# jacobstern/volume-viz

Hardware: AMD Instinct MI355X
Metric: Msamples/s (rays x steps), 1024^3 f32 volume @1080p (higher is better)
Workload: dtype f32

## Files before the change

### volume-viz_amd/csrc/vv_api.cpp

```cpp
#include "../../include/volviz.h"
#include "vv_kernels.h"

#include <hip/hip_runtime.h>
#include <climits>
#include <cmath>
#include <cstdio>
#include <cstdlib>
#include <cstring>
#include <string>
#include <algorithm>
#include <vector>

using namespace vv;

struct vv_knobs {
    int tile_log2w = -1, xcd_band = -1, unroll = -1, lds_reserve = -1, lds_reserve_phong = -1;
    int bricked = -1, zpair = -1, zfast = -1, force_big = 0;
    int block_w = -1, tail = -1, rect = -1, lpt = -1, lpt_run = -1, phong_bricks = -1;
    static int geti(const char *name, int dflt) { const char *e = getenv(name); return e ? atoi(e) : dflt; }
    void read()
    {
        tile_log2w = geti("VV_TILE_LOG2W", -1); xcd_band = geti("VV_XCD_BAND", -1); unroll = geti("VV_UNROLL", -1);
        lds_reserve = geti("VV_LDS_RESERVE", -1); lds_reserve_phong = geti("VV_LDS_RESERVE_PHONG", -1);
        bricked = geti("VV_BRICKED", -1); zpair = geti("VV_ZPAIR", -1);
        block_w = geti("VV_BLOCK_W", -1); tail = geti("VV_TAIL", -1);
        zfast = geti("VV_ZFAST", -1); force_big = getenv("VV_FORCE_BIG") != nullptr;
        rect = geti("VV_RECT", -1); lpt = geti("VV_LPT", -1); lpt_run = geti("VV_LPT_RUN", -1); phong_bricks = geti("VV_PHONG_BRICKS", -1);
    }
};

struct vv_context {
    int device = 0;
    vv_knobs knobs;
    hipStream_t stream = nullptr;
    hipEvent_t ev0 = nullptr, ev1 = nullptr;
    bool timed = false, time_frames = true;
    void *d_vol = nullptr; size_t vol_bytes = 0; int vtype = VV_VOXEL_U8; int nx = 0, ny = 0, nz = 0;
    size_t row_pitch = 0, slice_pitch = 0, alloc_bytes = 0;
    void *d_bricks = nullptr; bool bricks_valid = false, bricks_failed = false; uint32_t b_sy = 0, b_sz64 = 0; size_t bricks_bytes = 0;
    void *d_zpair = nullptr; bool zpair_valid = false; uint32_t zp_row = 0, zp_slab = 0; size_t zpair_bytes = 0;
    void *d_zfast = nullptr; bool zfast_valid = false, zfast_failed = false; uint32_t zf_row = 0; uint64_t zf_slice = 0; size_t zfast_bytes = 0;
    void *d_xpair = nullptr; bool xpair_valid = false, xpair_failed = false; uint32_t xp_row = 0, xp_slab = 0; size_t xpair_bytes = 0;
    size_t layout_budget_bytes = 0; bool build_in_render = true;
    unsigned long long frame_no = 0, last_used[4] = {0, 0, 0, 0};
    unsigned long long builds_in_render = 0;
    float last_density = 1e9f;
    float4 *d_tf = nullptr; bool tf_gray = false; bool have_tf = false;
    bool tf_alpha_unit = false;
    float *d_rad = nullptr; size_t rad_cap = 0;
// ... 594 lines not shown
    }
    launch_build_xpair(c->vtype, c->d_zfast, c->zf_row, c->zf_slice, c->d_xpair, c->nx, c->ny, c->nz, st);
    if (hipGetLastError() != hipSuccess ||
        hipMemsetAsync((char *)c->d_xpair + xb, 0, 32, st) != hipSuccess || hipStreamSynchronize(st) != hipSuccess) {
        (void)hipGetLastError(); (void)hipFree(c->d_xpair); c->d_xpair = nullptr; c->xpair_failed = true;
        return false;
    }
    c->xp_row = rb; c->xp_slab = sb; c->xpair_bytes = xb; c->xpair_valid = true;
    return true;
}

static VolumeView view_of(const vv_context *c)
{
    VolumeView V;
    const uint32_t vsz = c->vtype == VV_VOXEL_F32 ? 4 : 1;
    V.data = c->d_vol; V.nx = c->nx; V.ny = c->ny; V.nz = c->nz;
    (void)vsz;
    V.row_bytes = (uint32_t)c->row_pitch;
    V.slice_bytes = (uint32_t)c->slice_pitch;
    V.big = c->slice_pitch * (size_t)c->nz > (1ull << 32) || V.slice_bytes >= (1u << 24) || c->knobs.force_big;
    V.bricks = nullptr; V.b_sy = 0; V.b_sz64 = 0;
    V.zpair = nullptr; V.zp_row_bytes = 0; V.zp_slab_bytes = 0;
    V.zfast = nullptr; V.zf_row_bytes = 0; V.zf_slice_bytes = 0;
    return V;
}

static inline float vlen_h(float x, float y, float z) { return sqrtf(x * x + y * y + z * z); }

static int camera_basis(vv_context *c, FrameParams &P, const camera_params *cam, const vv_ray_source *rays, int W, int H)
{
    float lx = rays->look[0], ly = rays->look[1], lz = rays->look[2];
    float ll = vlen_h(lx, ly, lz);
    if (!(ll > 0.f)) return fail(c, VV_ERR_INVALID, "vv_render: look vector is zero");
    lx /= ll; ly /= ll; lz /= ll;
    float ux = rays->up[0], uy = rays->up[1], uz = rays->up[2];
    float sx = ly * uz - lz * uy, sy = lz * ux - lx * uz, sz = lx * uy - ly * ux;
    float sl = vlen_h(sx, sy, sz);
    if (!(sl > 0.f)) return fail(c, VV_ERR_INVALID, "vv_render: up vector is parallel to look");
    sx /= sl; sy /= sl; sz /= sl;
    float vx = sy * lz - sz * ly, vy = sz * lx - sx * lz, vz = sx * ly - sy * lx;
    float vl = vlen_h(vx, vy, vz);
    vx /= vl; vy /= vl; vz /= vl;
    P.look[0] = lx; P.look[1] = ly; P.look[2] = lz;
    P.side[0] = sx; P.side[1] = sy; P.side[2] = sz;
    P.up[0] = vx; P.up[1] = vy; P.up[2] = vz;
    float aspect = rays->aspect > 0.f ? rays->aspect : (float)W / (float)H;
// ... 73 lines not shown
    if (use_bricks) use_bricks = c->build_in_render ? ensure_bricks(c, st) : c->bricks_valid;
    if (use_bricks) {
        c->last_used[CP_BRICKS] = c->frame_no;
        A.V.bricks = c->d_bricks; A.V.b_sy = c->b_sy; A.V.b_sz64 = c->b_sz64;
        if (!k_unroll) A.unroll = 2;
        if (!k_reserve) A.lds_reserve = beyond_caches ? big_reserve : 36000;
    }
    bool use_zpair = !use_bricks && A.strips.tile_log2w == 5 && !shading->phongShading &&
                     (c->vtype == VV_VOXEL_U8 || c->vol_bytes <= (512ull << 20));
    if (K.zpair >= 0) use_zpair = K.zpair != 0 && !use_bricks;
    if (use_zfast) use_zpair = false;
    if (use_zpair) use_zpair = c->build_in_render ? ensure_zpair(c, st) : c->zpair_valid;
    if (use_zpair) { c->last_used[CP_ZPAIR] = c->frame_no; A.V.zpair = c->d_zpair; A.V.zp_row_bytes = c->zp_row; A.V.zp_slab_bytes = c->zp_slab; }
    A.xpair = false;
    if (use_zfast && !shading->phongShading && K.zpair != 0 && (c->vtype == VV_VOXEL_U8 || c->vol_bytes <= (512ull << 20)) &&
        (c->build_in_render ? ensure_xpair(c, st) : c->xpair_valid)) {
        A.xpair = true; c->last_used[CP_XPAIR] = c->frame_no;
        A.V.zpair = c->d_xpair; A.V.zp_row_bytes = c->xp_row; A.V.zp_slab_bytes = c->xp_slab;
    }
    c->builds_in_render += ((unsigned long long)c->bricks_valid + c->zpair_valid + c->zfast_valid + c->xpair_valid > builds_before)
                           ? ((unsigned long long)c->bricks_valid + c->zpair_valid + c->zfast_valid + c->xpair_valid - builds_before) : 0;
    A.lds_reserve_phong = c->vol_bytes > (8ull << 30) ? 40000 : ((beyond_caches && density > 3.5f && !use_bricks) ? 30000 : 13000);
    if (K.lds_reserve_phong >= 0 && K.lds_reserve_phong <= 146 * 1024) A.lds_reserve_phong = K.lds_reserve_phong;
    c->last_density = density;
    return beyond_caches;
}

static bool screen_rect(const MarchArgs &A, int W, int H, double *xmin, double *xmax, double *ymin, double *ymax)
{
    const FrameParams &P = A.P;
    double lo[2] = {INFINITY, INFINITY}, hi[2] = {-INFINITY, -INFINITY}, dmin = INFINITY, ext = 0.0;
    for (int a = 0; a < 3; ++a) ext = std::max(ext, (double)fabsf(P.cam_pos[a]) + (double)P.scale[a]);
    for (int k = 0; k < 8; ++k) {
        const double v[3] = {((k & 1) ? P.scale[0] : -P.scale[0]) - (double)P.cam_pos[0], ((k & 2) ? P.scale[1] : -P.scale[1]) - (double)P.cam_pos[1],
                             ((k & 4) ? P.scale[2] : -P.scale[2]) - (double)P.cam_pos[2]};
        const double depth = v[0] * P.look[0] + v[1] * P.look[1] + v[2] * P.look[2];
        if (!(depth > 1e-3 * ext)) return false;
        dmin = std::min(dmin, depth);
        const double sx = (v[0] * P.side[0] + v[1] * P.side[1] + v[2] * P.side[2]) / depth, sy = (v[0] * P.up[0] + v[1] * P.up[1] + v[2] * P.up[2]) / depth;
        const double px = (sx / P.tan_half_x + 1.0) * 0.5 * W - 0.5, py = (sy / P.tan_half_y + 1.0) * 0.5 * H - 0.5;
        lo[0] = std::min(lo[0], px); hi[0] = std::max(hi[0], px); lo[1] = std::min(lo[1], py); hi[1] = std::max(hi[1], py);
    }
    const double ang = 1e-4 * ext / dmin;
    const double mx = 1.0 + ang / (2.0 * P.tan_half_x / W), my = 1.0 + ang / (2.0 * P.tan_half_y / H);
    if (!std::isfinite(lo[0] + hi[0] + lo[1] + hi[1] + mx + my) || mx > W || my > H) return false;
    *xmin = lo[0] - mx; *xmax = hi[0] + mx; *ymin = lo[1] - my; *ymax = hi[1] + my;
// ... 213 lines not shown
        if (!whole) HIPCHK(c, hipMemcpyAsync(d_out, rgba_out, fb, hipMemcpyHostToDevice, st));
    }
    A.pixels = (uint32_t *)d_out;
    if (((uintptr_t)d_out & 3) != 0) return fail(c, VV_ERR_INVALID, "vv_render: output buffer must be 4-byte aligned");

    if (A.instr) HIPCHK(c, hipMemsetAsync(c->d_counter, 0, 16 * sizeof(unsigned long long), st));
#ifdef VV_TIMELINE
    { const char *e = getenv("VV_TIMELINE_PTR"); A.I.timeline = e ? (unsigned long long *)strtoull(e, nullptr, 0) : nullptr; }
#endif
    c->counter_valid = A.instr;
    {
        const int layout = A.xpair ? 5 : A.V.zfast ? 4 : (A.V.bricks ? 2 : (A.V.zpair ? 3 : ((A.V.big || (A.phong && beyond_caches)) ? 1 : 0)));
        const int v[8] = {A.strips.tile_log2w, A.strips.blk_log2w, A.unroll, A.phong ? A.lds_reserve_phong : A.lds_reserve, layout, have_basis ? 1 : 0,
                          (int)fminf(density * 1000.f, 2e9f), A.phong ? 1 : 0};
        memcpy(c->last_launch, v, sizeof v);
    }
    if (c->time_frames) HIPCHK(c, hipEventRecord(c->ev0, st));
    if (A.phong) {
        if (A.fill_outside) { A.rad_out = nullptr; launch_rad(A, st); }
        if (A.xpair) launch_raymarch_xpair(A, st); else if (A.V.zfast) launch_raymarch_zfast(A, st); else if (A.V.bricks) { if (beyond_caches) launch_raymarch_bricked(A, st); else launch_raymarch_bricked_cached(A, st); } else if (A.V.zpair) launch_raymarch_zpair(A, st); else if (A.V.big || beyond_caches) launch_raymarch_big(A, st); else launch_raymarch(A, st);
    } else if (A.strips.n_strips > 0) {
        if (W >= 2 && H >= 2) launch_rad(A, st);
        if (A.xpair) launch_raymarch_xpair(A, st);
        else if (A.V.zfast) launch_raymarch_zfast(A, st);
        else if (A.V.bricks) { if (beyond_caches) launch_raymarch_bricked(A, st); else launch_raymarch_bricked_cached(A, st); }
        else if (A.V.zpair) launch_raymarch_zpair(A, st);
        else if (A.V.big) launch_raymarch_big(A, st);
        else launch_raymarch(A, st);
    }
    if (c->time_frames) HIPCHK(c, hipEventRecord(c->ev1, st));
    HIPCHK(c, hipGetLastError());
    c->timed = c->time_frames;
    if (!out_on_device) {
        if (whole) HIPCHK(c, hipMemcpy2DAsync(rgba_out, (size_t)W * 4, d_out, (size_t)W * 4, (size_t)(W - 1) * 4, (size_t)(H - 1), hipMemcpyDeviceToHost, st));
        else HIPCHK(c, hipMemcpyAsync(rgba_out, d_out, fb, hipMemcpyDeviceToHost, st));
        HIPCHK(c, hipStreamSynchronize(st));
    } else if (!stream) {
        HIPCHK(c, hipStreamSynchronize(st));
    }
    return VV_OK;
}

int vv_first_pass(vv_context *c, int W, int H, const camera_params *cam, const vv_ray_source *rays,
                  uint8_t *front, uint8_t *back, int out_on_device, void *stream)
{
    if (!c) return fail(nullptr, VV_ERR_INVALID, "vv_first_pass: NULL context");
    if (!cam || !rays || !front || !back || W < 1 || H < 1) return fail(c, VV_ERR_INVALID, "vv_first_pass: bad argument");
    if (rays->mode != VV_RAYS_ANALYTIC) return fail(c, VV_ERR_INVALID, "vv_first_pass: needs an analytic ray source");
    for (int a = 0; a < 3; ++a)
// ... 211 lines not shown
```

### volume-viz_amd/csrc/vv_device.h

```cpp
#pragma once
#include <hip/hip_runtime.h>
#include <stdint.h>
#include "../../include/volviz.h"

namespace vv {

constexpr int   kCacheDepth = 32;
constexpr float kChunkSteps = 30.f;
constexpr int   kSlab = 14;
constexpr int   kBlock = 16;
constexpr float kSqrt3 = 1.73205081f;
constexpr float kEps = 1e-6f;

struct f3 { float x, y, z; };
__device__ __forceinline__ f3 mk3(float x, float y, float z) { return f3{x, y, z}; }

struct VolumeView {
    const void *data;
    int nx, ny, nz;
    uint32_t row_bytes;
    uint32_t slice_bytes;
    int big;
    const void *bricks;
    uint32_t b_sy;
    uint32_t b_sz64;
    const void *zpair;
    uint32_t zp_row_bytes;
    uint32_t zp_slab_bytes;
    const void *zfast;
    uint32_t zf_row_bytes;
    uint64_t zf_slice_bytes;
};
template <int VOXEL> struct BrickGeom;
#ifndef VV_BRICK_XLOG2
#define VV_BRICK_XLOG2 2
#endif
#ifndef VV_BRICK_HALO
#define VV_BRICK_HALO 1
#endif
#ifndef VV_BRICK_ZLOG2
#define VV_BRICK_ZLOG2 2
#endif
#ifndef VV_BRICK_X7
#define VV_BRICK_X7 0
#endif
#ifndef VV_BRICK_EXTRA
#define VV_BRICK_EXTRA 0
#endif
#if VV_BRICK_X7
template <> struct BrickGeom<VV_VOXEL_F32> { static constexpr uint32_t xlog2 = 0, bx = 7, halo = 1, row = 32,
                                             zlog2 = VV_BRICK_ZLOG2, bz = 1u << zlog2, rows = 4 * bz, brick = rows * row + VV_BRICK_EXTRA; };
#else
template <> struct BrickGeom<VV_VOXEL_F32> { static constexpr uint32_t xlog2 = VV_BRICK_XLOG2, bx = 1u << xlog2, halo = VV_BRICK_HALO, row = (bx + halo) * 4,
                                             zlog2 = VV_BRICK_ZLOG2, bz = 1u << zlog2, rows = 4 * bz, brick = rows * row; };
#endif
template <int VOXEL>
__device__ __forceinline__ uint32_t brick_x_offset(uint32_t ix)
{
    using G = BrickGeom<VOXEL>;
    if constexpr (VOXEL == VV_VOXEL_F32 && G::bx == 7) {
        const uint32_t q = (uint32_t)((float)ix * 0.142857149f);
        return __umul24(q, G::brick - 28u) + (ix << 2);
    } else if constexpr (VOXEL == VV_VOXEL_F32) {
        return __umul24(ix >> G::xlog2, G::brick) + ((ix & (G::bx - 1u)) << 2);
    } else {
        return (ix >> 2) * G::brick;
    }
}
template <> struct BrickGeom<VV_VOXEL_U8>  { static constexpr uint32_t xlog2 = 2, bx = 4, halo = 1, row = 8, zlog2 = 2, bz = 4, rows = 16, brick = 128; };
enum { LAYOUT_LINEAR = 0, LAYOUT_LINEAR_BIG = 1, LAYOUT_BRICKED = 2, LAYOUT_ZPAIR = 3, LAYOUT_ZFAST = 4 };

struct FrameParams {
    int W, H;
    int nbx, nby;
    int conflict_x, conflict_y;
    int rb, re, band, count, index;
    int slice_type;
    float slice_point[3], slice_normal[3];
    float cam_pos[3], scale[3], inv_scale[3];
    float step[3];
    float tan_fov_x, tan_fov_y;
    float ert_thr;
    int   ert_true;
    int   alpha_unit;
    int   max_chunks;
    int   safe_div;
    int ray_mode, quantize8;
    const uint8_t *front_img, *back_img; int img_w, img_h;
    float side[3], up[3], look[3];
    float tan_half_x, tan_half_y;
};

__device__ __forceinline__ int wave_min_i(int v) { for (int o = 32; o > 0; o >>= 1) v = min(v, __shfl_xor(v, o)); return v; }
// ... 126 lines not shown
}

__device__ __forceinline__ int chunk_count(float dist, float upper, float sstep)
{
#pragma clang fp contract(off)
    if (!(dist < upper)) return 0;
    float est = (upper - dist) / sstep;
    int n = est >= 30.f ? 30 : (est > 0.f ? (int)est : 0);
    while (n < 30 && !((float)(n + 1) * sstep + dist > upper)) ++n;
    while (n > 0 && ((float)n * sstep + dist > upper)) --n;
    if (sstep != sstep) n = 30;
    return n;
}
#pragma clang fp contract(fast)

typedef float  __attribute__((ext_vector_type(2), aligned(4))) float2u;
typedef unsigned short __attribute__((aligned(1))) ushort_u;

template <bool TEX8>
__device__ __forceinline__ float axis_coord(float x, float n, float nm1, uint32_t &i)
{
    float xb = __builtin_fmaf(x, n, -0.5f);
    xb = __builtin_amdgcn_fmed3f(xb, 0.0f, nm1);
    i = (uint32_t)xb;
    float a = __builtin_amdgcn_fractf(xb);
    if (TEX8) {
        const float magic = 49152.0f;
        float t = a + magic;
        a = t - magic;
    }
    return a;
}

template <int VOXEL> struct Corners;
template <> struct Corners<VV_VOXEL_F32> { float2u a, b, c, d; float wx, wy, wz; };
template <> struct Corners<VV_VOXEL_U8>  { uint32_t a0, a1, b0, b1, c0, c1, d0, d1, sh; float wx, wy, wz; };

template <int VOXEL>
__device__ __forceinline__ void load_rows(const char *b00, uint32_t row_bytes, uint32_t slice_bytes, uint32_t ix,
                                          uint32_t yz, Corners<VOXEL> &C)
{
    const char *b10 = b00 + row_bytes;
    const char *b01 = b00 + slice_bytes;
    const char *b11 = b01 + row_bytes;
    if constexpr (VOXEL == VV_VOXEL_F32) {
        const uint32_t off = ix * 4u + yz;
// ... 51 lines not shown
            const uint32_t ox = brick_x_offset<VOXEL>(ix);
            const uint32_t o0 = ox + oy0, o1 = ox + oy1;
            if constexpr (G::halo != 0) {
                C.a = *(const float2u *)(L0 + (o0 + zi0)); C.b = *(const float2u *)(L0 + (o1 + zi0));
                C.c = *(const float2u *)(L1 + (o0 + zi1)); C.d = *(const float2u *)(L1 + (o1 + zi1));
            } else {
                const uint32_t dx = (ix & (G::bx - 1u)) == G::bx - 1u ? G::brick - (G::bx - 1u) * 4u : 4u;
                const char *pa = L0 + (o0 + zi0), *pb = L0 + (o1 + zi0), *pc = L1 + (o0 + zi1), *pd = L1 + (o1 + zi1);
                const float a0 = *(const float *)pa, b0 = *(const float *)pb, c0 = *(const float *)pc, d0 = *(const float *)pd;
                const float a1 = *(const float *)(pa + dx), b1 = *(const float *)(pb + dx), c1 = *(const float *)(pc + dx), d1 = *(const float *)(pd + dx);
                C.a = {a0, a1}; C.b = {b0, b1}; C.c = {c0, c1}; C.d = {d0, d1};
            }
        } else {
            const uint32_t ox = (ix >> 2) * G::brick;
            const uint32_t o0 = ox + oy0, o1 = ox + oy1;
            C.sh = ix & 3u;
            const uint2 ra = *(const uint2 *)(L0 + (o0 + zi0)), rb = *(const uint2 *)(L0 + (o1 + zi0));
            const uint2 rc = *(const uint2 *)(L1 + (o0 + zi1)), rd = *(const uint2 *)(L1 + (o1 + zi1));
            C.a0 = ra.x; C.a1 = ra.y; C.b0 = rb.x; C.b1 = rb.y; C.c0 = rc.x; C.c1 = rc.y; C.d0 = rd.x; C.d1 = rd.y;
        }
    }
}

typedef float __attribute__((ext_vector_type(4), aligned(8))) float4u;
typedef float __attribute__((ext_vector_type(2))) float2v;
struct CornersZ { float wx, c000, c001, c100, c101, wy, c010, c011, c110, c111, wz; };

template <bool TEX8>
__device__ __forceinline__ void fetch_corners_zpair(const VolumeView &V, float px, float py, float pz, CornersZ &C)
{
    uint32_t ix, iy, iz;
    C.wx = axis_coord<TEX8>(px, (float)V.nx, (float)(V.nx - 1), ix);
    C.wy = axis_coord<TEX8>(py, (float)V.ny, (float)(V.ny - 1), iy);
    C.wz = axis_coord<TEX8>(pz, (float)V.nz, (float)(V.nz - 1), iz);
#ifdef VV_XPAIR
    const char *zb = (const char *)V.zpair + (uint64_t)ix * V.zp_slab_bytes;
    const uint32_t off = __umul24(iy, V.zp_row_bytes) + (iz << 3);
    const float4u r0 = *(const float4u *)(zb + off);
    const float4u r1 = *(const float4u *)(zb + off + V.zp_row_bytes);
    C.c000 = r0.x; C.c100 = r0.y; C.c001 = r0.z; C.c101 = r0.w;
    C.c010 = r1.x; C.c110 = r1.y; C.c011 = r1.z; C.c111 = r1.w;
#else
    const char *zb = (const char *)V.zpair + (uint64_t)iz * V.zp_slab_bytes;
    const uint32_t off = __umul24(iy, V.zp_row_bytes) + (ix << 3);
    const float4u r0 = *(const float4u *)(zb + off);
    const float4u r1 = *(const float4u *)(zb + off + V.zp_row_bytes);
// ... 193 lines not shown
```

### volume-viz_amd/csrc/vv_kernels.h

```cpp
#pragma once
#include <hip/hip_runtime.h>
#include "vv_device.h"

namespace vv {

struct StripMap { int y0, strips_per_band, band_stride_px, tile_log2w, n_strips, xcd_band;
                  int tail_batch;
                  int blk_log2w;
                  int tx0, wr, s0, s1;
                  const uint32_t *order; int order_run; };
struct PixelRect { int x0, x1, y0, y1; };

struct SlabMap  { int r0, band, band_stride, n_regular;
                  int gx0, wg, gs0, gs1; };

struct MarchArgs {
    FrameParams P;
    VolumeView  V;
    int V_type;
    bool tex8, gray, phong, instr;
    bool xpair;
    int lds_reserve;
    int unroll;
    int lds_reserve_phong;
    StripMap strips;
    PixelRect rect;
    bool fill_outside;
    uint32_t *order_out;
    SlabMap slabs;
    const float4 *tf;
    const float *rad;
    float *rad_out;
    uint32_t *pixels;
    unsigned long long *counter;
    InstrArgs I;
};

void launch_rad(const MarchArgs &a, hipStream_t s);
void launch_raymarch(const MarchArgs &a, hipStream_t s);
void launch_raymarch_big(const MarchArgs &a, hipStream_t s);
void launch_raymarch_bricked(const MarchArgs &a, hipStream_t s);
void launch_raymarch_bricked_cached(const MarchArgs &a, hipStream_t s);
void launch_raymarch_zpair(const MarchArgs &a, hipStream_t s);
void launch_raymarch_zfast(const MarchArgs &a, hipStream_t s);
void launch_raymarch_xpair(const MarchArgs &a, hipStream_t s);
void launch_build_xpair(int vtype, const void *zfast, uint32_t zf_row_bytes, uint64_t zf_slice_bytes, void *xpair, int nx, int ny, int nz, hipStream_t s);
void launch_build_zfast(int vtype, const void *vol, uint32_t row_pitch, uint64_t slice_pitch, void *out, uint32_t zf_row_bytes, uint64_t zf_slice_bytes, int nx, int ny, int nz, hipStream_t s);
size_t zpair_copy_bytes(int vtype, int nx, int ny, int nz, uint32_t *row_bytes, uint32_t *slab_bytes);
void launch_build_zpair(int vtype, const void *linear, size_t row_pitch, size_t slice_pitch, void *zpair, int nx, int ny, int nz, hipStream_t s);
void launch_repitch(const void *dense, void *pitched, size_t row_bytes , size_t ny, size_t nz,
                    size_t row_pitch, size_t slice_pitch, hipStream_t s);
size_t brick_copy_bytes(int vtype, int nx, int ny, int nz, uint32_t *sy, uint32_t *sz64);
void launch_build_bricks(int vtype, const void *linear, size_t row_pitch, size_t slice_pitch, void *bricks, int nx, int ny, int nz, hipStream_t s);
struct SliceArgs {
    VolumeView V; int V_type; bool tex8;
    float *buffer; size_t height, width;
    float dx, dy, dz; int orientation; int legacy;
    float scale[3];
    float trans[16]; int advanced;
};
void launch_slice(const SliceArgs &a, hipStream_t s);
void launch_first_pass(const FrameParams &P, uint32_t *front, uint32_t *back, hipStream_t s);

// ... 11 lines not shown
```

### volume-viz_amd/csrc/vv_raymarch.hip

```cpp
#include "vv_device.h"
#include "vv_kernels.h"

#if defined(VV_ZPAIR) && defined(VV_XPAIR)
#define VV_BIG_NS xpair
constexpr int kLayout = vv::LAYOUT_ZPAIR;
#elif defined(VV_ZPAIR)
#define VV_BIG_NS zpair
constexpr int kLayout = vv::LAYOUT_ZPAIR;
#elif defined(VV_BRICKED) && defined(VV_BRICKED_CACHED)
#define VV_BIG_NS brickc
constexpr int kLayout = vv::LAYOUT_BRICKED;
#elif defined(VV_BRICKED)
#define VV_BIG_NS brick
constexpr int kLayout = vv::LAYOUT_BRICKED;
#elif defined(VV_ZFAST)
#define VV_BIG_NS zfast
constexpr int kLayout = vv::LAYOUT_ZFAST;
#elif defined(VV_BIG_VOLUME)
#define VV_BIG_NS big
constexpr int kLayout = vv::LAYOUT_LINEAR_BIG;
#else
#define VV_BIG_NS small
constexpr int kLayout = vv::LAYOUT_LINEAR;
#endif

namespace vv {
namespace VV_BIG_NS {

template <int VOXEL> struct CornerSel { using type = Corners<VOXEL>; };
#ifdef VV_ZPAIR
template <> struct CornerSel<VV_VOXEL_F32> { using type = CornersZ; };
template <> struct CornerSel<VV_VOXEL_U8>  { using type = CornersZ8; };
#endif
template <int VOXEL, bool TEX8, class CT>
__device__ __forceinline__ void fetch_any(const VolumeView &V, float px, float py, float pz, CT &C)
{
#ifdef VV_ZPAIR
    fetch_corners_zpair<TEX8>(V, px, py, pz, C);
#else
    fetch_corners<VOXEL, TEX8, kLayout>(V, px, py, pz, C);
#endif
}

template <int VOXEL, bool TEX8>
__device__ __noinline__ void mark_sample_lines(const InstrArgs &I, const VolumeView &V, float px, float py, float pz)
{
    uint32_t ix, iy, iz;
    (void)axis_coord<TEX8>(px, (float)V.nx, (float)(V.nx - 1), ix);
    (void)axis_coord<TEX8>(py, (float)V.ny, (float)(V.ny - 1), iy);
    (void)axis_coord<TEX8>(pz, (float)V.nz, (float)(V.nz - 1), iz);
    constexpr bool F = VOXEL == VV_VOXEL_F32;
#if defined(VV_ZPAIR)
    const uint32_t rec = F ? 8u : 2u, bytes = F ? 16u : 4u;
#ifdef VV_XPAIR
    const uint64_t off = (uint64_t)ix * V.zp_slab_bytes + (uint64_t)iy * V.zp_row_bytes + (uint64_t)iz * rec;
#else
    const uint64_t off = (uint64_t)iz * V.zp_slab_bytes + (uint64_t)iy * V.zp_row_bytes + (uint64_t)ix * rec;
#endif
    mark_line_range(I, off, bytes); mark_line_range(I, off + V.zp_row_bytes, bytes);
#else
    if constexpr (kLayout == LAYOUT_LINEAR || kLayout == LAYOUT_LINEAR_BIG) {
        const uint64_t o = (uint64_t)iz * V.slice_bytes + (uint64_t)iy * V.row_bytes + (F ? ix * 4u : (ix & ~3u));
        mark_line_range(I, o, 8); mark_line_range(I, o + V.row_bytes, 8);
        mark_line_range(I, o + V.slice_bytes, 8); mark_line_range(I, o + V.slice_bytes + V.row_bytes, 8);
    } else if constexpr (kLayout == LAYOUT_ZFAST) {
// ... 156 lines not shown
        float length = vlen3(back.x - front.x, back.y - front.y, back.z - front.z);
        if (length < 0.001f) {
            write_zero = true;
        } else {
            float rd;
            if (P.W < 2 || P.H < 2) {
                rd = vlen3(front.x - P.cam_pos[0], front.y - P.cam_pos[1], front.z - P.cam_pos[2]);
            } else {
                int ox = owner_slab(x, P.W, P.nbx, P.conflict_x), oy = owner_slab(y, P.H, P.nby, P.conflict_y);
                rd = rad[oy * P.nbx + ox];
            }
            setup_ray(P, front, back, rd, r);
            alive = r.cut_return ? 0 : 1;
        }
    }
    if (!alive) { r.upper = -1.f; r.dist0 = 0.f; r.sstep = 1.f; r.origin = mk3(0, 0, 0); r.dir = r.origin; r.sdir = r.origin; }
    lds_tf[threadIdx.x] = tf_entry.x; lds_tf[256 + threadIdx.x] = tf_entry.y; lds_tf[512 + threadIdx.x] = tf_entry.z; lds_tf[768 + threadIdx.x] = tf_entry.w;
    __syncthreads();

    float dist = r.dist0;
    bool ert = false;
    const f3 sp = mk3(P.slice_point[0], P.slice_point[1], P.slice_point[2]);
    const f3 sn = mk3(P.slice_normal[0], P.slice_normal[1], P.slice_normal[2]);

    for (int chunk = 0; chunk < P.max_chunks && __any(dist < r.upper); ++chunk) {
        int n = chunk_count(dist, r.upper, r.sstep);
        if (ert && P.alpha_unit) n = min(n, 1);
        float px, py, pz;
        {
#pragma clang fp contract(off)
            px = r.origin.x + r.dir.x * dist;
            py = r.origin.y + r.dir.y * dist;
            pz = r.origin.z + r.dir.z * dist;
        }
        int nmax = 0;
#pragma unroll
        for (int bit = 16; bit > 0; bit >>= 1)
            if (__any(n >= (nmax | bit))) nmax |= bit;
        bool stop = false;
#ifndef VV_BRICKED
        if (nmax <= 1 && M.tail_batch) {
            float du[U], tx[U], ty[U], tz[U];
            int nu[U];
            typename CornerSel<VOXEL>::type C[U];
#pragma unroll
            for (int u = 0; u < U; ++u) {
#pragma clang fp contract(off)
                du[u] = u == 0 ? dist : du[u - 1] + r.sstep * kChunkSteps;
                nu[u] = u == 0 ? n : min(chunk_count(du[u], r.upper, r.sstep), 1);
                if (chunk + u >= P.max_chunks) nu[u] = 0;
                float qx = r.origin.x + r.dir.x * du[u], qy = r.origin.y + r.dir.y * du[u], qz = r.origin.z + r.dir.z * du[u];
                qx += r.sdir.x; qy += r.sdir.y; qz += r.sdir.z;
                tx[u] = __builtin_fmaf(qx - 0.5f, P.inv_scale[0], 0.5f);
                ty[u] = __builtin_fmaf(qy - 0.5f, P.inv_scale[1], 0.5f);
                tz[u] = __builtin_fmaf(qz - 0.5f, P.inv_scale[2], 0.5f);
                fetch_any<VOXEL, TEX8>(V, tx[u], ty[u], tz[u], C[u]);
            }
            __builtin_amdgcn_sched_barrier(0);
            if (INSTR) slots += 64ull * U;
#pragma unroll
            for (int u = 0; u < U; ++u) {
                const uint32_t k = classify_index<VOXEL>(C[u], tx[u], ty[u], tz[u]);
                const bool live = nu[u] >= 1 && !(P.ert_true && ert);
                float cr, cg, cb, ca;
                ca = lds_tf[768 + k];
                cr = lds_tf[k];
                if (GRAY) { cg = cb = cr; }
                else { cg = lds_tf[256 + k]; cb = lds_tf[512 + k]; }
                if (SLICE == SLICE_PLANE) {
#pragma clang fp contract(off)
                    float vd = 1.f * r.sstep + du[u];
                    float vx = r.origin.x + r.dir.x * vd, vy = r.origin.y + r.dir.y * vd, vz = r.origin.z + r.dir.z * vd;
                    float d = fabsf(sn.x * (vx - sp.x) + sn.y * (vy - sp.y) + sn.z * (vz - sp.z));
                    if (d < .01f) cr = fmaxf(0.f, fminf(cr + (.01f - d) * 100.f, 1.f));
                }
                if (INSTR) {
                    const bool inv = bounds_check(tx[u], ty[u], tz[u]);
                    if (live) {
                        executed++;
                        if (I.bricks && inv) mark_bricks(I.bricks, V, tx[u], ty[u], tz[u]);
                    }
                    if ((I.lines || I.pairs) && (I.lines_all || (live && inv))) mark_sample_lines<VOXEL, TEX8>(I, V, tx[u], ty[u], tz[u]);
                }
                {
#pragma clang fp contract(off)
                    const float bf = (live && ca > kEps) ? ca * (1.f - res_a) : 0.f;
                    res_r = res_r + cr * bf;
                    if (!GRAY) { res_g = res_g + cg * bf; res_b = res_b + cb * bf; }
                    res_a = res_a + bf;
                }
                ert = ert || (live && res_a > P.ert_thr);
            }
            if (P.ert_true && ert) r.upper = -1.f;
            {
#pragma clang fp contract(off)
                dist = du[U - 1] + r.sstep * kChunkSteps;
            }
            chunk += U - 1;
            continue;
        }
#endif
        if (INSTR) slots += (unsigned long long)((nmax + U - 1) / U * U) * 64ull;
        for (int i0 = 1; i0 <= nmax; i0 += U) {
            float tx[U], ty[U], tz[U];
            typename CornerSel<VOXEL>::type C[U];
#pragma unroll
            for (int u = 0; u < U; ++u) {
                px += r.sdir.x; py += r.sdir.y; pz += r.sdir.z;
                tx[u] = __builtin_fmaf(px - 0.5f, P.inv_scale[0], 0.5f);
                ty[u] = __builtin_fmaf(py - 0.5f, P.inv_scale[1], 0.5f);
                tz[u] = __builtin_fmaf(pz - 0.5f, P.inv_scale[2], 0.5f);
                fetch_any<VOXEL, TEX8>(V, tx[u], ty[u], tz[u], C[u]);
            }
            __builtin_amdgcn_sched_barrier(0);
            uint32_t idx[U];
#pragma unroll
            for (int u = 0; u < U; ++u) idx[u] = classify_index<VOXEL>(C[u], tx[u], ty[u], tz[u]);
#pragma unroll
            for (int u = 0; u < U; ++u) {
                const int i = i0 + u;
                const bool live = i <= n && !stop;
                float cr, cg, cb, ca;
                ca = lds_tf[768 + idx[u]];
                cr = lds_tf[idx[u]];
                if (GRAY) { cg = cb = cr; }
                else { cg = lds_tf[256 + idx[u]]; cb = lds_tf[512 + idx[u]]; }
                if (SLICE == SLICE_PLANE) {
#pragma clang fp contract(off)
                    float vd = (float)i * r.sstep + dist;
                    float vx = r.origin.x + r.dir.x * vd, vy = r.origin.y + r.dir.y * vd, vz = r.origin.z + r.dir.z * vd;
                    float d = fabsf(sn.x * (vx - sp.x) + sn.y * (vy - sp.y) + sn.z * (vz - sp.z));
                    if (d < .01f) cr = fmaxf(0.f, fminf(cr + (.01f - d) * 100.f, 1.f));
                }
                if (INSTR) {
                    const bool inv = bounds_check(tx[u], ty[u], tz[u]);
                    if (live) {
                        executed++;
                        if (I.bricks && inv) mark_bricks(I.bricks, V, tx[u], ty[u], tz[u]);
                    }
                    if ((I.lines || I.pairs) && (I.lines_all || (live && inv))) mark_sample_lines<VOXEL, TEX8>(I, V, tx[u], ty[u], tz[u]);
                }
                {
#pragma clang fp contract(off)
                    const float bf = (live && ca > kEps) ? ca * (1.f - res_a) : 0.f;
                    res_r = res_r + cr * bf;
                    if (!GRAY) { res_g = res_g + cg * bf; res_b = res_b + cb * bf; }
                    res_a = res_a + bf;
                }
                const bool hit = live && res_a > P.ert_thr;
                stop = stop || hit;
                ert = ert || hit;
            }
        }
        if (P.ert_true && ert) r.upper = -1.f;
        {
#pragma clang fp contract(off)
            dist += r.sstep * kChunkSteps;
        }
    }

    if (in_frame) {
        if (GRAY) { res_g = res_r; res_b = res_r; }
        pixels[(size_t)y * P.W + x] = write_zero ? 0u : pack_rgba(res_r, res_g, res_b, res_a);
    }
#ifdef VV_TIMELINE
    {
        const bool any_live = __any(alive) != 0;
        if (I.timeline && threadIdx.x == 0) {
            unsigned long long *t = I.timeline + 4ull * blockIdx.x;
            t[0] = tl0; t[1] = wall_clock64(); t[2] = ((unsigned long long)strip << 16) | (unsigned)tile_x;
            t[3] = (__builtin_amdgcn_s_getreg((3 << 11) | 20) & 15u) | (any_live ? 256u : 0u) | ((unsigned long long)__builtin_amdgcn_s_getreg((31 << 11) | 4) << 16);
        }
    }
#endif
    if (INSTR) {
        for (int o = 32; o > 0; o >>= 1) executed += __shfl_down(executed, o);
        if (lane == 0 && executed) atomicAdd(counter, executed);
        if (lane == 0 && slots) atomicAdd(counter + 1, slots);
        if (kLayout == LAYOUT_BRICKED && lane == 0 && executed) atomicAdd(counter + 2, 1ull);
        if (kLayout == LAYOUT_ZPAIR && lane == 0 && executed) atomicAdd(counter + 3, 1ull);
    }
}

__device__ __forceinline__ float ph_div_core(float n, float d)
{
    const float y0 = __builtin_amdgcn_rcpf(d);
    const float e = __builtin_fmaf(-d, y0, 1.0f);
    const float y = __builtin_fmaf(e, y0, y0);
    const float q0 = n * y;
    const float r0 = __builtin_fmaf(-d, q0, n);
    const float q1 = __builtin_fmaf(r0, y, q0);
    const float r1 = __builtin_fmaf(-d, q1, n);
    return __builtin_fmaf(r1, y, q1);
}
__device__ __forceinline__ float ph_sqrt_core(float x)
{
    const float s0 = __builtin_amdgcn_sqrtf(x);
    const float sm = __uint_as_float(__float_as_uint(s0) - 1u), sp = __uint_as_float(__float_as_uint(s0) + 1u);
    const float t1 = __builtin_fmaf(-sm, s0, x);
    float s = (0.f >= t1) ? sm : s0;
    const float t2 = __builtin_fmaf(-sp, s0, x);
    s = (0.f < t2) ? sp : s;
    return s;
// ... 249 lines not shown
    dim3 grid(nblocks);
    if (a.unroll == 3)
        hipLaunchKernelGGL((march_kernel<SLICE, VOXEL, TEX8, GRAY, INSTR, 3>), grid, dim3(256), (size_t)a.lds_reserve, s,
                           a.P, a.V, a.tf, a.rad, a.pixels, a.counter, a.I, a.strips);
    else
        hipLaunchKernelGGL((march_kernel<SLICE, VOXEL, TEX8, GRAY, INSTR, 2>), grid, dim3(256), (size_t)a.lds_reserve, s,
                           a.P, a.V, a.tf, a.rad, a.pixels, a.counter, a.I, a.strips);
}
template <int SLICE, int VOXEL, bool TEX8, bool INSTR>
static void launch_phong(const MarchArgs &a, hipStream_t s)
{
    const int rows = a.slabs.gs1 - a.slabs.gs0 + 1;
    constexpr int BAND = VV_PHONG_BAND;
    if (a.slabs.wg <= 0) return;
    dim3 grid((unsigned)(((rows + 8 * BAND - 1) / (8 * BAND)) * 8 * BAND * a.slabs.wg));
    hipLaunchKernelGGL((march_phong_kernel<SLICE, VOXEL, TEX8, INSTR>), grid, dim3(256), (size_t)a.lds_reserve_phong, s,
                       a.P, a.V, a.tf, a.slabs, a.pixels, a.counter, a.I);
}

template <int SLICE, int VOXEL, bool TEX8>
static void dispatch3(const MarchArgs &a, hipStream_t s)
{
    if (a.phong) {
        if (a.instr) launch_phong<SLICE, VOXEL, TEX8, true>(a, s); else launch_phong<SLICE, VOXEL, TEX8, false>(a, s);
        return;
    }
    const bool gray = a.gray && SLICE != SLICE_PLANE;
    if (gray) { if (a.instr) launch_march<SLICE, VOXEL, TEX8, true, true>(a, s); else launch_march<SLICE, VOXEL, TEX8, true, false>(a, s); }
    else      { if (a.instr) launch_march<SLICE, VOXEL, TEX8, false, true>(a, s); else launch_march<SLICE, VOXEL, TEX8, false, false>(a, s); }
}
template <int SLICE>
static void dispatch2(const MarchArgs &a, hipStream_t s)
{
    if (a.V_type == VV_VOXEL_F32) { if (a.tex8) dispatch3<SLICE, VV_VOXEL_F32, true>(a, s); else dispatch3<SLICE, VV_VOXEL_F32, false>(a, s); }
    else                          { if (a.tex8) dispatch3<SLICE, VV_VOXEL_U8,  true>(a, s); else dispatch3<SLICE, VV_VOXEL_U8,  false>(a, s); }
}

static void launch_rad_impl(const MarchArgs &a, hipStream_t s)
{
    dim3 grid((unsigned)((a.P.nbx * a.P.nby + 3) / 4) + (a.order_out ? 1u : 0u));
    hipLaunchKernelGGL(rad_kernel, grid, dim3(256), 0, s, a.P, a.rad_out, a.rect, a.pixels, a.strips, a.order_out);
}

static void launch_raymarch_impl(const MarchArgs &a, hipStream_t s)
{
    switch (a.P.slice_type) {
    case SLICE_PLANE:     dispatch2<SLICE_PLANE>(a, s); break;
    case SLICE_PLANE_CUT: dispatch2<SLICE_PLANE_CUT>(a, s); break;
    default:              dispatch2<SLICE_NONE>(a, s); break;
    }
}

}

#if defined(VV_ZPAIR) && defined(VV_XPAIR)
void launch_raymarch_xpair(const MarchArgs &a, hipStream_t s) { xpair::launch_raymarch_impl(a, s); }
#elif defined(VV_ZPAIR)
void launch_raymarch_zpair(const MarchArgs &a, hipStream_t s) { zpair::launch_raymarch_impl(a, s); }
#elif defined(VV_BRICKED) && defined(VV_BRICKED_CACHED)
void launch_raymarch_bricked_cached(const MarchArgs &a, hipStream_t s) { brickc::launch_raymarch_impl(a, s); }
#elif defined(VV_BRICKED)
void launch_raymarch_bricked(const MarchArgs &a, hipStream_t s) { brick::launch_raymarch_impl(a, s); }
#elif defined(VV_ZFAST)
void launch_raymarch_zfast(const MarchArgs &a, hipStream_t s) { zfast::launch_raymarch_impl(a, s); }
#elif defined(VV_BIG_VOLUME)
void launch_raymarch_big(const MarchArgs &a, hipStream_t s) { big::launch_raymarch_impl(a, s); }
#else
void launch_rad(const MarchArgs &a, hipStream_t s) { small::launch_rad_impl(a, s); }
void launch_raymarch(const MarchArgs &a, hipStream_t s) { small::launch_raymarch_impl(a, s); }
#endif

}
```

Measured before the change: 220,800.

## Add 32-bit addressing window kernels for big volumes with per-chunk window selection

Adds new raymarch kernel variants (linear and zfast layouts) that split a volume larger than 4 GiB into two overlapping windows, each addressable with 32-bit offsets from a base pointer. Per chunk, a wave-wide ballot checks whether every lane's samples fall inside one window. If so, it uses cheap 32-bit umul24 addressing, otherwise it falls back to the wide 64-bit fetch. The goal is to remove the 64-bit address arithmetic cost of the big-volume path. In exchange it adds ballot and window-selection overhead and extra code size, and phong shading is disabled in these kernels.

```diff
diff --git a/volume-viz_amd/csrc/vv_api.cpp b/volume-viz_amd/csrc/vv_api.cpp
--- a/volume-viz_amd/csrc/vv_api.cpp
+++ b/volume-viz_amd/csrc/vv_api.cpp
@@ -15,7 +15,7 @@
 
 struct vv_knobs {
     int tile_log2w = -1, xcd_band = -1, unroll = -1, lds_reserve = -1, lds_reserve_phong = -1;
-    int bricked = -1, zpair = -1, zfast = -1, force_big = 0;
+    int bricked = -1, zpair = -1, zfast = -1, force_big = 0, win32 = -1, win_slices = -1;
     int block_w = -1, tail = -1, rect = -1, lpt = -1, lpt_run = -1, phong_bricks = -1;
     static int geti(const char *name, int dflt) { const char *e = getenv(name); return e ? atoi(e) : dflt; }
     void read()
@@ -25,6 +25,7 @@
         bricked = geti("VV_BRICKED", -1); zpair = geti("VV_ZPAIR", -1);
         block_w = geti("VV_BLOCK_W", -1); tail = geti("VV_TAIL", -1);
         zfast = geti("VV_ZFAST", -1); force_big = getenv("VV_FORCE_BIG") != nullptr;
+        win32 = geti("VV_WIN32", -1); win_slices = geti("VV_WIN32_SLICES", -1);
         rect = geti("VV_RECT", -1); lpt = geti("VV_LPT", -1); lpt_run = geti("VV_LPT_RUN", -1); phong_bricks = geti("VV_PHONG_BRICKS", -1);
     }
 };
@@ -665,6 +666,7 @@
     V.bricks = nullptr; V.b_sy = 0; V.b_sz64 = 0;
     V.zpair = nullptr; V.zp_row_bytes = 0; V.zp_slab_bytes = 0;
     V.zfast = nullptr; V.zf_row_bytes = 0; V.zf_slice_bytes = 0;
+    V.win_n = 0;
     return V;
 }
 
@@ -784,6 +786,18 @@
                            ? ((unsigned long long)c->bricks_valid + c->zpair_valid + c->zfast_valid + c->xpair_valid - builds_before) : 0;
     A.lds_reserve_phong = c->vol_bytes > (8ull << 30) ? 40000 : ((beyond_caches && density > 3.5f && !use_bricks) ? 30000 : 13000);
     if (K.lds_reserve_phong >= 0 && K.lds_reserve_phong <= 146 * 1024) A.lds_reserve_phong = K.lds_reserve_phong;
+    A.V.win_n = 0;
+    if (!shading->phongShading && !A.V.bricks && !A.V.zpair && !A.xpair && !K.force_big && K.win32 != 0) {
+        const bool zf = A.V.zfast != nullptr;
+        const uint64_t pitch = zf ? A.V.zf_slice_bytes : (uint64_t)A.V.slice_bytes;
+        const int n = zf ? c->nx : c->nz;
+        const bool beyond = zf ? false : A.V.big;
+        if ((beyond || K.win32 == 1) && pitch > 0 && pitch < (1u << 24)) {
+            int w = (int)std::min<uint64_t>((1ull << 32) / pitch, (uint64_t)n);
+            if (K.win_slices > 0) w = std::min(w, K.win_slices);
+            if (2 * w >= n) A.V.win_n = w;
+        }
+    }
     c->last_density = density;
     return beyond_caches;
 }
@@ -1043,9 +1057,10 @@
     } else if (A.strips.n_strips > 0) {
         if (W >= 2 && H >= 2) launch_rad(A, st);
         if (A.xpair) launch_raymarch_xpair(A, st);
-        else if (A.V.zfast) launch_raymarch_zfast(A, st);
+        else if (A.V.zfast) { if (A.V.win_n) launch_raymarch_zfast_win(A, st); else launch_raymarch_zfast(A, st); }
         else if (A.V.bricks) { if (beyond_caches) launch_raymarch_bricked(A, st); else launch_raymarch_bricked_cached(A, st); }
         else if (A.V.zpair) launch_raymarch_zpair(A, st);
+        else if (A.V.win_n) launch_raymarch_win(A, st);
         else if (A.V.big) launch_raymarch_big(A, st);
         else launch_raymarch(A, st);
     }
diff --git a/volume-viz_amd/csrc/vv_device.h b/volume-viz_amd/csrc/vv_device.h
--- a/volume-viz_amd/csrc/vv_device.h
+++ b/volume-viz_amd/csrc/vv_device.h
@@ -30,6 +30,7 @@
     const void *zfast;
     uint32_t zf_row_bytes;
     uint64_t zf_slice_bytes;
+    int win_n;
 };
 template <int VOXEL> struct BrickGeom;
 #ifndef VV_BRICK_XLOG2
@@ -68,7 +69,7 @@
     }
 }
 template <> struct BrickGeom<VV_VOXEL_U8>  { static constexpr uint32_t xlog2 = 2, bx = 4, halo = 1, row = 8, zlog2 = 2, bz = 4, rows = 16, brick = 128; };
-enum { LAYOUT_LINEAR = 0, LAYOUT_LINEAR_BIG = 1, LAYOUT_BRICKED = 2, LAYOUT_ZPAIR = 3, LAYOUT_ZFAST = 4 };
+enum { LAYOUT_LINEAR = 0, LAYOUT_LINEAR_BIG = 1, LAYOUT_BRICKED = 2, LAYOUT_ZPAIR = 3, LAYOUT_ZFAST = 4, LAYOUT_LINEAR_WIN = 5, LAYOUT_ZFAST_WIN = 6 };
 
 struct FrameParams {
     int W, H;
@@ -241,6 +242,20 @@
 {
     float xb = __builtin_fmaf(x, n, -0.5f);
     xb = __builtin_amdgcn_fmed3f(xb, 0.0f, nm1);
+    i = (uint32_t)xb;
+    float a = __builtin_amdgcn_fractf(xb);
+    if (TEX8) {
+        const float magic = 49152.0f;
+        float t = a + magic;
+        a = t - magic;
+    }
+    return a;
+}
+
+template <bool TEX8>
+__device__ __forceinline__ float axis_coord_win(float x, float n, float lo, float hi, uint32_t &i)
+{
+    float xb = __builtin_amdgcn_fmed3f(__builtin_fmaf(x, n, -0.5f), lo, hi);
     i = (uint32_t)xb;
     float a = __builtin_amdgcn_fractf(xb);
     if (TEX8) {
@@ -338,6 +353,34 @@
     }
 }
 
+struct Win { const char *base; uint32_t adj; float lo, hi; };
+
+template <int VOXEL, bool TEX8, int LAYOUT>
+__device__ __forceinline__ void fetch_corners_win(const VolumeView &V, const Win &W, float px, float py, float pz, Corners<VOXEL> &C)
+{
+    uint32_t ix, iy, iz;
+    if constexpr (LAYOUT == LAYOUT_LINEAR_WIN) {
+        C.wx = axis_coord<TEX8>(px, (float)V.nx, (float)(V.nx - 1), ix);
+        C.wy = axis_coord<TEX8>(py, (float)V.ny, (float)(V.ny - 1), iy);
+        C.wz = axis_coord_win<TEX8>(pz, (float)V.nz, W.lo, W.hi, iz);
+        load_rows<VOXEL>(W.base, V.row_bytes, V.slice_bytes, ix, __umul24(iy, V.row_bytes) + __umul24(iz, V.slice_bytes) + W.adj, C);
+    } else {
+        C.wx = axis_coord_win<TEX8>(px, (float)V.nx, W.lo, W.hi, ix);
+        C.wy = axis_coord<TEX8>(py, (float)V.ny, (float)(V.ny - 1), iy);
+        C.wz = axis_coord<TEX8>(pz, (float)V.nz, (float)(V.nz - 1), iz);
+        const uint32_t sb = (uint32_t)V.zf_slice_bytes;
+        const uint32_t yx = __umul24(iy, V.zf_row_bytes) + __umul24(ix, sb) + W.adj;
+        if constexpr (VOXEL == VV_VOXEL_F32) {
+            Corners<VOXEL> T;
+            load_rows<VOXEL>(W.base, V.zf_row_bytes, sb, iz, yx, T);
+            C.a.x = T.a.x; C.a.y = T.c.x; C.b.x = T.b.x; C.b.y = T.d.x;
+            C.c.x = T.a.y; C.c.y = T.c.y; C.d.x = T.b.y; C.d.y = T.d.y;
+        } else {
+            load_rows<VOXEL>(W.base, V.zf_row_bytes, sb, iz, yx, C);
+        }
+    }
+}
+
 typedef float __attribute__((ext_vector_type(4), aligned(8))) float4u;
 typedef float __attribute__((ext_vector_type(2))) float2v;
 struct CornersZ { float wx, c000, c001, c100, c101, wy, c010, c011, c110, c111, wz; };
diff --git a/volume-viz_amd/csrc/vv_kernels.h b/volume-viz_amd/csrc/vv_kernels.h
--- a/volume-viz_amd/csrc/vv_kernels.h
+++ b/volume-viz_amd/csrc/vv_kernels.h
@@ -39,6 +39,8 @@
 void launch_rad(const MarchArgs &a, hipStream_t s);
 void launch_raymarch(const MarchArgs &a, hipStream_t s);
 void launch_raymarch_big(const MarchArgs &a, hipStream_t s);
+void launch_raymarch_win(const MarchArgs &a, hipStream_t s);
+void launch_raymarch_zfast_win(const MarchArgs &a, hipStream_t s);
 void launch_raymarch_bricked(const MarchArgs &a, hipStream_t s);
 void launch_raymarch_bricked_cached(const MarchArgs &a, hipStream_t s);
 void launch_raymarch_zpair(const MarchArgs &a, hipStream_t s);
diff --git a/volume-viz_amd/csrc/vv_raymarch.hip b/volume-viz_amd/csrc/vv_raymarch.hip
--- a/volume-viz_amd/csrc/vv_raymarch.hip
+++ b/volume-viz_amd/csrc/vv_raymarch.hip
@@ -1,7 +1,16 @@
 #include "vv_device.h"
 #include "vv_kernels.h"
-
-#if defined(VV_ZPAIR) && defined(VV_XPAIR)
+#include <type_traits>
+
+#if defined(VV_WINDOW32) && defined(VV_ZFAST)
+#define VV_BIG_NS zfwin
+constexpr int kLayout = vv::LAYOUT_ZFAST;
+constexpr int kWinLayout = vv::LAYOUT_ZFAST_WIN;
+#elif defined(VV_WINDOW32)
+#define VV_BIG_NS win
+constexpr int kLayout = vv::LAYOUT_LINEAR_BIG;
+constexpr int kWinLayout = vv::LAYOUT_LINEAR_WIN;
+#elif defined(VV_ZPAIR) && defined(VV_XPAIR)
 #define VV_BIG_NS xpair
 constexpr int kLayout = vv::LAYOUT_ZPAIR;
 #elif defined(VV_ZPAIR)
@@ -41,6 +50,7 @@
     fetch_corners<VOXEL, TEX8, kLayout>(V, px, py, pz, C);
 #endif
 }
+template <bool WIDE> struct FetchSel {};
 
 template <int VOXEL, bool TEX8>
 __device__ __noinline__ void mark_sample_lines(const InstrArgs &I, const VolumeView &V, float px, float py, float pz)
@@ -243,6 +253,26 @@
     bool ert = false;
     const f3 sp = mk3(P.slice_point[0], P.slice_point[1], P.slice_point[2]);
     const f3 sn = mk3(P.slice_normal[0], P.slice_normal[1], P.slice_normal[2]);
+#ifdef VV_WINDOW32
+#ifndef VV_WIN_TAIL
+#define VV_WIN_TAIL 0
+#endif
+    constexpr int WA = kLayout == LAYOUT_ZFAST ? 0 : 2;
+    const int wn = WA == 0 ? V.nx : V.nz, w1 = wn - V.win_n;
+    const uint32_t wpitch = WA == 0 ? (uint32_t)V.zf_slice_bytes : V.slice_bytes;
+    const char *wdata = (const char *)(WA == 0 ? V.zfast : V.data);
+    const float w0_hi = (float)(V.win_n - 1), w1_lo = (float)w1, w1_hi = (float)(wn - 1), wnf = (float)wn;
+    const char *const w1_base = wdata + (uint64_t)w1 * wpitch;
+    const uint32_t w1_adj = 0u - (uint32_t)w1 * wpitch;
+    unsigned long long n_win = 0, n_wide = 0;
+    auto win_coord = [&](float p) { return __builtin_fmaf(__builtin_fmaf(p - 0.5f, P.inv_scale[WA], 0.5f), wnf, -0.5f); };
+    auto pick_window = [&](bool used, float lo, float hi) {
+        if (__builtin_amdgcn_ballot_w64(used && !(hi < w0_hi)) == 0ull) return 0;
+        if (__builtin_amdgcn_ballot_w64(used && !(lo >= w1_lo)) == 0ull) return 1;
+        return -1;
+    };
+    auto window_of = [&](int w) { return w == 0 ? Win{wdata, 0u, 0.f, w0_hi} : Win{w1_base, w1_adj, w1_lo, w1_hi}; };
+#endif
 
     for (int chunk = 0; chunk < P.max_chunks && __any(dist < r.upper); ++chunk) {
         int n = chunk_count(dist, r.upper, r.sstep);
@@ -275,8 +305,26 @@
                 tx[u] = __builtin_fmaf(qx - 0.5f, P.inv_scale[0], 0.5f);
                 ty[u] = __builtin_fmaf(qy - 0.5f, P.inv_scale[1], 0.5f);
                 tz[u] = __builtin_fmaf(qz - 0.5f, P.inv_scale[2], 0.5f);
+#if !defined(VV_WINDOW32) || !VV_WIN_TAIL
                 fetch_any<VOXEL, TEX8>(V, tx[u], ty[u], tz[u], C[u]);
-            }
+#endif
+            }
+#if defined(VV_WINDOW32) && VV_WIN_TAIL
+            {
+                const float *tw = WA == 0 ? tx : tz;
+                const float c0 = __builtin_fmaf(tw[0], wnf, -0.5f), c1 = __builtin_fmaf(tw[U - 1], wnf, -0.5f);
+                const int w = pick_window(n > 0, fminf(c0, c1), fmaxf(c0, c1));
+                if (w >= 0) {
+                    const Win Wn = window_of(w);
+#pragma unroll
+                    for (int u = 0; u < U; ++u) fetch_corners_win<VOXEL, TEX8, kWinLayout>(V, Wn, tx[u], ty[u], tz[u], C[u]);
+                } else {
+#pragma unroll
+                    for (int u = 0; u < U; ++u) fetch_any<VOXEL, TEX8>(V, tx[u], ty[u], tz[u], C[u]);
+                }
+                if (INSTR) { if (w >= 0) n_win++; else n_wide++; }
+            }
+#endif
             __builtin_amdgcn_sched_barrier(0);
             if (INSTR) slots += 64ull * U;
 #pragma unroll
@@ -322,6 +370,11 @@
         }
 #endif
         if (INSTR) slots += (unsigned long long)((nmax + U - 1) / U * U) * 64ull;
+#ifdef VV_WINDOW32
+        Win Wn{};
+#endif
+        auto trips = [&](auto sel) {
+        [[maybe_unused]] constexpr bool WIDE = std::is_same<decltype(sel), FetchSel<true>>::value;
         for (int i0 = 1; i0 <= nmax; i0 += U) {
             float tx[U], ty[U], tz[U];
             typename CornerSel<VOXEL>::type C[U];
@@ -331,6 +384,9 @@
                 tx[u] = __builtin_fmaf(px - 0.5f, P.inv_scale[0], 0.5f);
                 ty[u] = __builtin_fmaf(py - 0.5f, P.inv_scale[1], 0.5f);
                 tz[u] = __builtin_fmaf(pz - 0.5f, P.inv_scale[2], 0.5f);
+#ifdef VV_WINDOW32
+                if constexpr (!WIDE) fetch_corners_win<VOXEL, TEX8, kWinLayout>(V, Wn, tx[u], ty[u], tz[u], C[u]); else
+#endif
                 fetch_any<VOXEL, TEX8>(V, tx[u], ty[u], tz[u], C[u]);
             }
             __builtin_amdgcn_sched_barrier(0);
@@ -373,6 +429,20 @@
                 ert = ert || hit;
             }
         }
+        };
+#ifdef VV_WINDOW32
+        {
+            const float p0 = WA == 0 ? px : pz, e = 30.f * (WA == 0 ? r.sdir.x : r.sdir.z);
+            const float err = __builtin_fmaf(fabsf(p0) + fabsf(e), 0x1p-16f, 0x1p-60f);
+            const float ca = win_coord(p0 + fminf(e, 0.f) - err), cb = win_coord(p0 + fmaxf(e, 0.f) + err);
+            const int w = pick_window(n > 0, fminf(ca, cb), fmaxf(ca, cb));
+            if (INSTR) { if (w >= 0) n_win++; else n_wide++; }
+            if (w >= 0) { Wn = window_of(w); trips(FetchSel<false>{}); }
+            else trips(FetchSel<true>{});
+        }
+#else
+        trips(FetchSel<true>{});
+#endif
         if (P.ert_true && ert) r.upper = -1.f;
         {
 #pragma clang fp contract(off)
@@ -400,6 +470,10 @@
         if (lane == 0 && slots) atomicAdd(counter + 1, slots);
         if (kLayout == LAYOUT_BRICKED && lane == 0 && executed) atomicAdd(counter + 2, 1ull);
         if (kLayout == LAYOUT_ZPAIR && lane == 0 && executed) atomicAdd(counter + 3, 1ull);
+#ifdef VV_WINDOW32
+        if (lane == 0 && n_wide) atomicAdd(counter + 4, n_wide);
+        if (lane == 0 && n_win) atomicAdd(counter + 5, n_win);
+#endif
     }
 }
 
@@ -695,7 +769,9 @@
 static void dispatch3(const MarchArgs &a, hipStream_t s)
 {
     if (a.phong) {
+#ifndef VV_WINDOW32
         if (a.instr) launch_phong<SLICE, VOXEL, TEX8, true>(a, s); else launch_phong<SLICE, VOXEL, TEX8, false>(a, s);
+#endif
         return;
     }
     const bool gray = a.gray && SLICE != SLICE_PLANE;
@@ -726,7 +802,11 @@
 
 }
 
-#if defined(VV_ZPAIR) && defined(VV_XPAIR)
+#if defined(VV_WINDOW32) && defined(VV_ZFAST)
+void launch_raymarch_zfast_win(const MarchArgs &a, hipStream_t s) { zfwin::launch_raymarch_impl(a, s); }
+#elif defined(VV_WINDOW32)
+void launch_raymarch_win(const MarchArgs &a, hipStream_t s) { win::launch_raymarch_impl(a, s); }
+#elif defined(VV_ZPAIR) && defined(VV_XPAIR)
 void launch_raymarch_xpair(const MarchArgs &a, hipStream_t s) { xpair::launch_raymarch_impl(a, s); }
 #elif defined(VV_ZPAIR)
 void launch_raymarch_zpair(const MarchArgs &a, hipStream_t s) { zpair::launch_raymarch_impl(a, s); }
diff --git a/volume-viz_amd/csrc/vv_raymarch_win.hip b/volume-viz_amd/csrc/vv_raymarch_win.hip
--- /dev/null
+++ b/volume-viz_amd/csrc/vv_raymarch_win.hip
@@ -0,0 +1,2 @@
+#define VV_WINDOW32 1
+#include "vv_raymarch.hip"
diff --git a/volume-viz_amd/csrc/vv_raymarch_zfast_win.hip b/volume-viz_amd/csrc/vv_raymarch_zfast_win.hip
--- /dev/null
+++ b/volume-viz_amd/csrc/vv_raymarch_zfast_win.hip
@@ -0,0 +1,3 @@
+#define VV_ZFAST 1
+#define VV_WINDOW32 1
+#include "vv_raymarch.hip"
```

Result: no change. 219,700, median of 3 (-0.5%).
